# kuwt/edge_alignment

Hardware: NVIDIA B200
Metric: frame-pair alignments/sec at 640x480 (higher is better)
Workload: dtype f32+f64

## Files before the change

### edge_alignment_b200/csrc/ea_cabi.cu

```cuda
#include <cstdarg>
#include <cstdio>
#include <cstdlib>
#include <cmath>
#include <algorithm>
#include <cstring>
#include <mutex>
#include <vector>
#include <new>

#include "ea_internal.h"

thread_local std::string g_ea_err;
int ea_fail(int code, const char* fmt, ...) {
  char buf[512];
  va_list ap;
  va_start(ap, fmt);
  vsnprintf(buf, sizeof buf, fmt, ap);
  va_end(ap);
  g_ea_err = buf;
  return code;
}

int ea_ensure_tmp(ea_context* c, size_t bytes) {
  if (c->tmp_cap >= bytes) return EA_OK;
// ... 8 lines not shown
int ea_abi_version(void) { return EA_ABI_VERSION; }
const char* ea_last_error(void) { return g_ea_err.c_str(); }

int ea_create(int device, ea_context** out) {
  if (!out) return ea_fail(EA_ERR_INVALID_ARG, "ea_create: out is null");
  *out = nullptr;
  int n = 0;
  cudaError_t e = cudaGetDeviceCount(&n);
  if (e != cudaSuccess || n == 0)
    return ea_fail(EA_ERR_NO_DEVICE, "ea_create: no CUDA device (%s); this library has no CPU fallback", cudaGetErrorString(e));
  if (device < 0 || device >= n) return ea_fail(EA_ERR_INVALID_ARG, "ea_create: device %d out of range [0,%d)", device, n);
  CU(cudaSetDevice(device));
  cudaDeviceProp prop;
  CU(cudaGetDeviceProperties(&prop, device));
  if (prop.major < 10) return ea_fail(EA_ERR_NO_DEVICE, "ea_create: device %d is sm_%d%d; this build is sm_100a only", device, prop.major, prop.minor);
  ea_context* c = new (std::nothrow) ea_context();
  if (!c) return ea_fail(EA_ERR_INVALID_ARG, "out of host memory");
  struct Guard { ea_context* c; ~Guard() { if (c) ea_destroy(c); } } guard{c};
  c->device = device; c->sm_count = prop.multiProcessorCount; c->cc_major = prop.major; c->cc_minor = prop.minor;
  CU(cudaStreamCreateWithFlags(&c->stream, cudaStreamNonBlocking));
  c->own_stream = true;
  CU(cudaMalloc(&c->d_pose, 7 * sizeof(double)));
  CU(cudaMalloc(&c->d_failed, sizeof(int)));
  CU(cudaMalloc(&c->d_work, sizeof(int)));
  CU(cudaMalloc(&c->d_sums, size_t(1024) * EA_SUMS * sizeof(double)));
  {
    const char* h = getenv("EA_SOLVE_HELPERS");
    if (!(h && h[0] == '0')) {
      c->boards_bytes = ea_help_boards_bytes(c->sm_count);
      CU(cudaMalloc(&c->d_boards, c->boards_bytes));
    }
  }
  if (getenv("EA_SOLVE_DEBUG")) {
    CU(cudaMalloc(&c->d_debug, size_t(1024) * 6 * sizeof(unsigned long long)));
    CU(cudaMemset(c->d_debug, 0, size_t(1024) * 6 * sizeof(unsigned long long)));
  }
  guard.c = nullptr;
  *out = c;
  return EA_OK;
}
int ea_destroy(ea_context* c) {
  if (!c) return EA_OK;
  cudaSetDevice(c->device);
  cudaStreamSynchronize(c->stream);
  if (c->d_debug && c->debug_launches > 0) {
    const double n = double(c->debug_launches);
    fprintf(stderr, "[EA_SOLVE_DEBUG] %ld launches; per launch, mean over CTAs, kcycles of thread 0: eval %.1f  wait+totals %.1f  LM %.1f  wait2 %.1f  lifetime %.1f; evaluations %.1f\n",
            c->debug_launches, c->debug_sum[0] / n / 1e3, c->debug_sum[1] / n / 1e3, c->debug_sum[2] / n / 1e3, c->debug_sum[3] / n / 1e3, c->debug_sum[5] / n / 1e3, c->debug_sum[4] / n);
  }
  cudaFree(c->d_debug); cudaFree(c->d_boards); cudaFree(c->d_views);
  for (int k = 0; k < EA_PREP_MAX_PARTS; ++k) {
    if (c->prep_pipe.aux[k]) { cudaStreamSynchronize(c->prep_pipe.aux[k]); cudaStreamDestroy(c->prep_pipe.aux[k]); }
    if (c->prep_pipe.ev_front[k]) cudaEventDestroy(c->prep_pipe.ev_front[k]);
    if (c->prep_pipe.ev_dt[k]) cudaEventDestroy(c->prep_pipe.ev_dt[k]);
  }
  cudaFree(c->d_pose); cudaFree(c->d_failed); cudaFree(c->d_work); cudaFree(c->d_sums); cudaFree(c->d_idx); cudaFree(c->d_tmp);
  if (c->own_stream) cudaStreamDestroy(c->stream);
  delete c;
  return EA_OK;
}
int ea_sync(ea_context* c) {
  if (!c) return ea_fail(EA_ERR_INVALID_ARG, "null context");
  CU(cudaStreamSynchronize(c->stream));
  return EA_OK;
}
int ea_set_stream(ea_context* c, void* s) {
  if (!c) return ea_fail(EA_ERR_INVALID_ARG, "null context");
  if (c->own_stream) { cudaStreamSynchronize(c->stream); cudaStreamDestroy(c->stream); c->own_stream = false; }
  c->stream = static_cast<cudaStream_t>(s);
  return EA_OK;
}
int ea_device_info(ea_context* c, int* sm, int* maj, int* min_) {
  if (!c) return ea_fail(EA_ERR_INVALID_ARG, "null context");
  if (sm) *sm = c->sm_count;
  if (maj) *maj = c->cc_major;
  if (min_) *min_ = c->cc_minor;
  return EA_OK;
}
int ea_host_alloc(void** p, size_t bytes) {
  if (!p) return ea_fail(EA_ERR_INVALID_ARG, "null pointer");
  CU(cudaHostAlloc(p, bytes, cudaHostAllocDefault));
// ... 553 lines not shown
  if (e != cudaSuccess) return ea_fail(EA_ERR_CUDA, "gather probe: %s", cudaGetErrorString(e));
  CU(cudaEventElapsedTime(ms, ev.a, ev.b));
  std::vector<int32_t> slots(static_cast<size_t>(n));
  CU(cudaMemcpy(slots.data(), d_ref_slots, size_t(n) * sizeof(int32_t), cudaMemcpyDeviceToHost));
  std::vector<int> npts(size_t(ref->n_slots) * EA_MAX_LEVELS);
  CU(cudaMemcpy(npts.data(), ref->d_npts, npts.size() * sizeof(int), cudaMemcpyDeviceToHost));
  double total = 0.0;
  for (int i = 0; i < n; ++i) total += std::min(npts[size_t(slots[size_t(i)]) * EA_MAX_LEVELS + level], ref->lv[level].cap);
  *point_gathers = total * repeats;
  return EA_OK;
}

int ea_solve_batch_device_ordered(ea_context* c, int n, ea_frameset* ref, const int32_t* d_ref_slots, ea_frameset* now,
                                  const int32_t* d_now_slots, double* d_poses7, const int32_t* d_pose_index,
                                  const int32_t* d_order, const ea_solve_params* sp, ea_summary* d_summaries, bool tail_helpers) {
  if (!c || !d_ref_slots || !d_now_slots || !d_poses7) return ea_fail(EA_ERR_INVALID_ARG, "null argument");
  if (n <= 0) return EA_OK;
  EaSolveArgs A;
  int cluster = 0;
  int rc = fill_solve_args(c, ref, now, sp, A, &cluster);
  if (rc) return rc;
  CU(cudaSetDevice(c->device));
  A.ref_slots = d_ref_slots; A.now_slots = d_now_slots; A.pose_index = d_pose_index; A.poses = d_poses7;
  A.summaries = d_summaries; A.n_pairs = n; A.work_counter = c->d_work; A.order = d_order;
  EaProfileScope prof(c, 1);
  cudaError_t e;
  A.trace = c->d_trace; A.trace_count = c->d_trace_count; A.trace_cap = c->trace_cap;
  if (cluster == 0) cluster = auto_cluster(c, n, 0);
  A.debug = c->d_debug;
  A.boards = tail_helpers ? static_cast<EaHelpBoard*>(c->d_boards) : nullptr;
  e = ea_launch_solve_batch(A, cluster, c->sm_count, c->stream);
  if (c->d_debug && e == cudaSuccess) {
    const int grid = std::min(n, c->sm_count);
    std::vector<unsigned long long> h(size_t(grid) * 6);
    cudaStreamSynchronize(c->stream);
    cudaMemcpy(h.data(), c->d_debug, h.size() * sizeof(unsigned long long), cudaMemcpyDeviceToHost);
    for (int k = 0; k < 6; ++k) { double sum = 0; for (int b = 0; b < grid; ++b) sum += double(h[size_t(b) * 6 + k]); c->debug_sum[k] += sum / grid; }
    {
      std::vector<double> life(static_cast<size_t>(grid));
      double mean = 0.0;
      for (int b = 0; b < grid; ++b) { life[size_t(b)] = double(h[size_t(b) * 6 + 5]); mean += life[size_t(b)] / grid; }
      std::sort(life.begin(), life.end());
      if (c->debug_launches % 7 == 3)
        fprintf(stderr, "[EA_SOLVE_DEBUG] launch %ld: owner lifetimes (kcycles) mean %.0f  p50 %.0f  p75 %.0f  p90 %.0f  p97 %.0f  max %.0f\n", c->debug_launches,
                mean / 1e3, life[size_t(grid / 2)] / 1e3, life[size_t(grid * 3 / 4)] / 1e3, life[size_t(grid * 9 / 10)] / 1e3, life[size_t(grid * 97 / 100)] / 1e3, life[size_t(grid - 1)] / 1e3);
    }
    c->debug_launches++;
  }
  c->launches++;
  if (e != cudaSuccess) return ea_fail(EA_ERR_CUDA, "solve launch: %s", cudaGetErrorString(e));
  return EA_OK;
}
extern "C" {

int ea_solve_batch(ea_context* c, int n, ea_frameset* ref, const int32_t* ref_slots, ea_frameset* now, const int32_t* now_slots,
                   double* poses7, const ea_solve_params* sp, ea_summary* summaries) {
  if (!c || !ref_slots || !now_slots || !poses7) return ea_fail(EA_ERR_INVALID_ARG, "null argument");
  if (n <= 0) return EA_OK;
  int rc = check_pairable(ref, now);
  if (!rc) rc = check_slots(ref, std::min(n, ref->n_slots), ref_slots);
  if (rc) return rc;
  for (int i = 0; i < n; ++i) {
    if (ref_slots[i] < 0 || ref_slots[i] >= ref->n_slots || now_slots[i] < 0 || now_slots[i] >= now->n_slots)
      return ea_fail(EA_ERR_INVALID_ARG, "pair %d: slot out of range", i);
    double q2 = 0;
    for (int k = 0; k < 4; ++k) q2 += poses7[i * 7 + k] * poses7[i * 7 + k];
    if (!(q2 > 0.999999 && q2 < 1.000001)) return ea_fail(EA_ERR_INVALID_ARG, "pair %d: quaternion is not unit (|q|^2=%g)", i, q2);
  }
  CU(cudaSetDevice(c->device));
  const int L = ref->p.n_levels;
  const size_t bytes = size_t(n) * (2 * sizeof(int32_t) + 7 * sizeof(double)) + size_t(n) * L * sizeof(ea_summary) + 64;
  rc = ea_ensure_tmp(c, bytes);
  if (rc) return rc;
  char* base = (char*)c->d_tmp;
// ... 46 lines not shown
```

### edge_alignment_b200/csrc/ea_internal.h

```cpp
#pragma once
#include <cuda_runtime.h>

#include <string>
#include <vector>

#include "ea_device.cuh"

#include "ea_solve.cuh"

#define EA_TRACE_DOUBLES 6

struct EaSolveArgs {
  const EaLevelDesc* ref_desc;
  const EaLevelDesc* now_desc;
  const int32_t* ref_slots;
  const int32_t* now_slots;
  const int32_t* pose_index;
  const int32_t* order;
  double* poses;
  int* work_counter;
  struct EaHelpBoard* boards;
  unsigned long long* debug;
  ea_summary* summaries;
  double* trace;
  int* trace_count;
  int trace_cap;
  int n_pairs, n_levels, coarsest, finest;
  double inv_depth_scale;
  EaLevelGeom ref_geom[EA_MAX_LEVELS];
  EaLevelGeom now_geom[EA_MAX_LEVELS];
  int ref_cap[EA_MAX_LEVELS];
  ea_solve_params sp;
  EaEvalConsts loss;
};

cudaError_t ea_launch_solve_batch(const EaSolveArgs& A, int cluster_size, int sm_count, cudaStream_t stream);
size_t ea_help_boards_bytes(int sm_count);
cudaError_t ea_launch_gather_probe(const EaSolveArgs& A, int level, int slices, int repeats, float* d_sink, cudaStream_t stream);
int ea_probe_gather_device(ea_context* c, int n, ea_frameset* ref, const int32_t* d_ref_slots, ea_frameset* now, const int32_t* d_now_slots,
                           const double* d_poses7, int level, int repeats, float* ms, double* point_gathers);
cudaError_t ea_launch_eval_points(const EaLevelDesc& rd, const EaLevelDesc& nd, const EaLevelGeom& rg,
                                  const EaLevelGeom& ng, double inv_depth_scale, const ea_solve_params& sp,
                                  const double* d_pose7, int n_res, double* d_raw, double* d_res, double* d_jac,
// ... 36 lines not shown
  int zero_to_one;
  float depth_one;
  EaCannyCfg canny;
  EaScratch scratch;
};
#define EA_PREP_MAX_PARTS 4
struct EaPrepPipe {
  cudaStream_t aux[EA_PREP_MAX_PARTS] = {};
  cudaEvent_t ev_front[EA_PREP_MAX_PARTS] = {}, ev_dt[EA_PREP_MAX_PARTS] = {};
  bool ready = false;
};
cudaError_t ea_launch_preprocess(const EaPrepArgs& A, int sm_count, cudaStream_t stream, int* launches, const EaPrepPipe* pipe = nullptr);
__host__ __device__ inline float* ea_dt_origin(const EaPrepLevel& L, int slot) {
  return L.dt + size_t(slot) * L.dt_slot + size_t(EA_DT_PAD) * L.dt_pitch + EA_DT_PAD;
}
cudaError_t ea_launch_dt_normalized_copy(const float* origin, int pitch, const float2* affine, int w, int h, float* out, cudaStream_t stream);
cudaError_t ea_launch_dt_import(const float* src, float* origin, int w, int h, int pitch, cudaStream_t stream);
cudaError_t ea_launch_dt_fill_pad(const EaPrepLevel& L, const int32_t* d_slots, int n, cudaStream_t stream);
cudaError_t ea_launch_canny_level(const EaPrepArgs& A, int l, const uint8_t* bgr, const void* depth, size_t frame_stride_px,
                                  bool slot_indexed, const EaCannyCfg& cfg, const EaScratch& S, cudaStream_t stream, int* launches);
cudaError_t ea_launch_exact_edt_level(const EaPrepArgs& A, int l, const EaScratch& S, cudaStream_t stream, int* launches);
cudaError_t ea_launch_unpack_mask(const uint32_t* bits, int w, int h, int words, int median, uint8_t* out,
                                  cudaStream_t stream);

struct ea_context {
  int device = 0, sm_count = 0, cc_major = 0, cc_minor = 0;
  cudaStream_t stream = nullptr;
  bool own_stream = false;
  int64_t launches = 0;
  double* d_pose = nullptr;
  int* d_failed = nullptr;
  int* d_work = nullptr;
  void* d_boards = nullptr; size_t boards_bytes = 0;
  unsigned long long* d_debug = nullptr; double debug_sum[6] = {0, 0, 0, 0, 0, 0}; long debug_launches = 0;
  double* d_sums = nullptr;
  int32_t* d_idx = nullptr;
  size_t idx_cap = 0;
  void* d_tmp = nullptr;
  size_t tmp_cap = 0;
  void* d_views = nullptr; size_t views_cap = 0;
  EaPrepPipe prep_pipe;
  bool profile = false;
  double* d_trace = nullptr; int* d_trace_count = nullptr; int trace_cap = 0;
  std::vector<cudaEvent_t> ev[2];
};
struct EaProfileScope {
  ea_context* c; int kind; cudaStream_t s;
  EaProfileScope(ea_context* c_, int kind_, cudaStream_t s_ = nullptr) : c(c_), kind(kind_), s(s_ ? s_ : c_->stream) {
    if (c->profile) { cudaEvent_t e; cudaEventCreate(&e); cudaEventRecord(e, s); c->ev[kind].push_back(e); }
  }
  ~EaProfileScope() {
    if (c->profile) { cudaEvent_t e; cudaEventCreate(&e); cudaEventRecord(e, s); c->ev[kind].push_back(e); }
  }
};

struct ea_frameset {
  ea_context* ctx = nullptr;
  ea_frame_params p;
  int n_slots = 0;
  EaPrepLevel lv[EA_MAX_LEVELS];
  EaLevelGeom geom[EA_MAX_LEVELS];
  EaLevelDesc* d_desc = nullptr;
  std::vector<EaLevelDesc> h_desc;
  int* d_npts = nullptr;
  unsigned* d_minmax = nullptr;
  float2* d_affine = nullptr;
  int* d_overflow = nullptr;
// ... 45 lines not shown
```

### edge_alignment_b200/csrc/ea_solve.cu

```cuda
#include <cooperative_groups.h>

#include "ea_internal.h"
#include <cstdlib>

#include "ea_solve.cuh"

namespace cg = cooperative_groups;

#define EA_SOLVE_WARPS (EA_SOLVE_THREADS / 32)
#ifndef EA_SOLVE_MIN_CTAS
#define EA_SOLVE_MIN_CTAS 1
#endif
#define EA_CMD_EXIT 2

struct EaMsg {
  const void* pts;
  const float* dt;
  float2 affine;
  int n_res, level, pts_mode, cmd;
  int rev;
  int same;
  int nh, pad;
  EaPose P;
};
#define EA_MSG_FIXED_WORDS 5
static_assert(sizeof(EaMsg) % 8 == 0, "EaMsg is copied as 8-byte words");

#define EA_MAX_HELPERS (EA_MAX_CHUNKS - 1)
#define EA_BOARD_EXIT (~0ull)
#define EA_BOARD_SPIN_LIMIT (1ll << 22)
struct EaHelpBoard {
  unsigned long long word;
  int n_helpers;
  int busy;
  unsigned long long done[EA_MAX_HELPERS];
  double chunk[EA_MAX_CHUNKS][32];
  EaMsg msg;
};

struct alignas(2 * EA_STAGE_SLOT * 8) EaSolveSmem {
  uint2 stage[2][EA_STAGE_SLOT];
  EaSolveArgs args;
  EaMsg msg[2];
  double part[EA_MAX_CHUNKS][EA_SOLVE_WARPS][EA_NSUM];
  double cpart[EA_MAX_CHUNKS][EA_SOLVE_WARPS];
  double sums[EA_SUMS + 3];
  double cluster_sums[8][EA_SUMS + 3];
  EaLmState lm;
  int pair, level, truncated;
  unsigned long long help_epoch;
  int help_owner, help_index, help_fail;
  long long dbg[6], dbg_t, dbg_t0;
};

template <bool INL>
__device__ __forceinline__ void ea_boss_next_impl(const EaSolveArgs& A, EaSolveSmem& S, EaMsg& out, bool new_pair_needed) {
  for (;;) {
    if (new_pair_needed) {
      const int ticket = atomicAdd(A.work_counter, 1);
      if (ticket >= A.n_pairs) { out.cmd = EA_CMD_EXIT; S.pair = -1; return; }
      const int pair = A.order ? A.order[ticket] : ticket;
      S.pair = pair; S.level = A.coarsest;
      const int pi = A.pose_index ? A.pose_index[pair] : pair;
#pragma unroll 1
      for (int i = 0; i < 7; ++i) S.lm.x[i] = A.poses[size_t(pi) * 7 + i];
      new_pair_needed = false;
    }
    const int pair = S.pair, level = S.level;
    if (level < A.finest) {
      const int pi = A.pose_index ? A.pose_index[pair] : pair;
#pragma unroll 1
      for (int i = 0; i < 7; ++i) A.poses[size_t(pi) * 7 + i] = S.lm.x[i];
      new_pair_needed = true;
      continue;
    }
    const EaLevelDesc rd = A.ref_desc[size_t(A.ref_slots[pair]) * EA_MAX_LEVELS + level];
    const EaLevelDesc nd = A.now_desc[size_t(A.now_slots[pair]) * EA_MAX_LEVELS + level];
    const int n_pts = min(*rd.n_pts, A.ref_cap[level]);
    const int n_res = (n_pts + A.sp.point_stride - 1) / A.sp.point_stride;
    S.truncated = *rd.truncated;
    if (n_res == 0) {
      if (A.summaries) { ea_summary z = {}; z.termination = EA_TERM_SKIPPED_NO_POINTS; A.summaries[size_t(pair) * A.n_levels + level] = z; }
      S.level = level - 1;
      continue;
    }
    EaLmState& L = S.lm;
    L.phase = 0; L.iter = 0; L.accepted = 0; L.rejected = 0; L.invalid_run = 0; L.evals = 0; L.term = EA_TERM_NONE;
#pragma unroll 1
    for (int i = 0; i < 7; ++i) L.cand[i] = L.x[i];
    if (rd.pts_mode == EA_POINTS_XYZ) ea_pose_setup<true>(L.cand, A.ref_geom[level], A.now_geom[level], out.P);
    else ea_pose_setup<false>(L.cand, A.ref_geom[level], A.now_geom[level], out.P);
    out.pts = rd.pts; out.dt = nd.dt - ea_dt_origin_offset(nd.w); out.affine = *nd.dt_affine; out.n_res = n_res; out.level = level; out.pts_mode = rd.pts_mode; out.cmd = EA_CMD_EVAL; out.rev = 0; out.same = 0; out.nh = 0; out.pad = 0;
    return;
  }
}

__device__ __noinline__ void ea_boss_next(const EaSolveArgs& A, EaSolveSmem& S, EaMsg& out, bool new_pair_needed) { ea_boss_next_impl<false>(A, S, out, new_pair_needed); }

__device__ __forceinline__ void ea_boss_step_warp(const EaSolveArgs& A, EaSolveSmem& S, const EaMsg& cur, EaMsg& out, const int lane) {
  const int acc0 = S.lm.accepted, rej0 = S.lm.rejected;
#ifdef EA_LM_PROFILE
  const long long t_in = clock64();
#endif
  const int cmd = ea_lm_advance_warp(S.lm, S.sums, A.sp, lane);
#ifdef EA_LM_PROFILE
  __syncwarp();
  if (lane == 0) { S.lm.prof[6] += clock64() - t_in; S.lm.prof[7] += 1; }
  __syncwarp();
#endif
  if (A.trace && lane == 0) {
    const int k = (*A.trace_count)++;
    if (k < A.trace_cap) {
      double* r = A.trace + size_t(k) * EA_TRACE_DOUBLES;
      r[0] = cur.level; r[1] = S.lm.accepted + S.lm.rejected; r[2] = S.lm.cost; r[3] = S.sums[28]; r[4] = S.lm.radius;
      r[5] = S.lm.accepted > acc0 ? 1.0 : (S.lm.rejected > rej0 ? 0.0 : -1.0);
    }
  }
  if (cmd == EA_CMD_EVAL) {
    EaPose P;
    if (cur.pts_mode == EA_POINTS_XYZ) ea_pose_setup<true>(S.lm.cand, A.ref_geom[cur.level], A.now_geom[cur.level], P);
    else ea_pose_setup<false>(S.lm.cand, A.ref_geom[cur.level], A.now_geom[cur.level], P);
    if (lane < EA_MSG_FIXED_WORDS) reinterpret_cast<unsigned long long*>(&out)[lane] = reinterpret_cast<const unsigned long long*>(&cur)[lane];
    if (lane == 5) { out.rev = S.lm.evals & 1; out.same = 1; out.nh = 0; out.pad = 0; }
    if (lane == 0) out.P = P;
    __syncwarp();
    return;
  }
  if (lane == 0) {
    if (A.summaries) {
      const EaLmState& L = S.lm;
      ea_summary z;
      z.termination = L.term; z.iterations = L.iter; z.accepted = L.accepted; z.rejected = L.rejected;
      z.n_residuals = cur.n_res; z.evaluations = L.evals; z.initial_cost = L.initial_cost; z.final_cost = L.cost;
      z.truncated = S.truncated; z.reserved = 0;
      A.summaries[size_t(S.pair) * A.n_levels + cur.level] = z;
    }
    S.level = cur.level - 1;
    ea_boss_next(A, S, out, false);
  }
  __syncwarp();
}


__device__ __forceinline__ unsigned long long ea_ld_acquire(const unsigned long long* p) {
  unsigned long long v;
  asm volatile("ld.acquire.gpu.global.u64 %0, [%1];" : "=l"(v) : "l"(p) : "memory");
  return v;
}
__device__ __forceinline__ void ea_st_release(unsigned long long* p, unsigned long long v) {
  asm volatile("st.release.gpu.global.u64 [%0], %1;" ::"l"(p), "l"(v) : "memory");
}

template <int THREADS>
__device__ __forceinline__ void ea_eval_chunks(const EaSolveArgs& A, EaSolveSmem& S, const EaMsg& M, const EaPose& P, const int cb, const int ce,
                                               const int chunk, const bool pre_valid, const bool chain_next_eval) {
  const EaLevelGeom& ng = A.now_geom[M.level];
  const bool rev = EA_ALTERNATE_SWEEP && M.rev, nrev = EA_ALTERNATE_SWEEP ? !rev : rev;
  const int lo = cb * chunk, hi = min(ce * chunk, M.n_res);
  if (M.pts_mode == EA_POINTS_XYZ)
    ea_eval_slice<true, THREADS>(M.pts, M.dt, M.affine, ng, A.inv_depth_scale, A.loss, A.sp.point_stride, P, lo, hi, S.part[cb], S.cpart[cb], rev, nullptr, false, false, false,
                                 chunk / THREADS, THREADS / 32);
  else
    ea_eval_slice<false, THREADS>(M.pts, M.dt, M.affine, ng, A.inv_depth_scale, A.loss, A.sp.point_stride, P, lo, hi, S.part[cb], S.cpart[cb], rev, &S.stage[0][0], pre_valid, chain_next_eval, nrev,
                                  chunk / THREADS, THREADS / 32);
}

template <int THREADS, bool CLUSTER>
__global__ void __launch_bounds__(THREADS, EA_SOLVE_MIN_CTAS) ea_k_solve_batch(const __grid_constant__ EaSolveArgs A) {
  __shared__ EaSolveSmem S;
  cg::cluster_group cluster = cg::this_cluster();
  const unsigned crank = CLUSTER ? cluster.block_rank() : 0u;
  const unsigned csize = CLUSTER ? cluster.num_blocks() : 1u;
  const int tid = threadIdx.x, lane = tid & 31, warp = tid >> 5;
  const bool boss = (crank == 0 && tid == 0);
  const bool helpers_on = !CLUSTER && A.boards != nullptr;
  EaHelpBoard* const my_board = helpers_on ? A.boards + blockIdx.x : nullptr;
  auto sync_all = [&]() { if (CLUSTER) cluster.sync(); else __syncthreads(); };
  auto publish = [&](const EaMsg& m, unsigned slot) {
    for (unsigned r = 0; r < csize; ++r) {
      EaSolveSmem* Sr = CLUSTER ? cluster.map_shared_rank(&S, r) : &S;
      Sr->msg[slot] = m;
    }
  };
  unsigned g = 0;
  if (tid == 0) S.args = A;
  __syncthreads();
  if (boss) {
    EaMsg m;
    S.help_epoch = 0; S.help_fail = 0;
    ea_boss_next(S.args, S, m, true);
    if (helpers_on && m.cmd != EA_CMD_EXIT) { *reinterpret_cast<volatile int*>(&my_board->busy) = 1; __threadfence(); }
    publish(m, 0);
  }
  sync_all();
  const bool dbg_on = A.debug != nullptr && tid == 0;
  if (dbg_on) { for (int k = 0; k < 6; ++k) S.dbg[k] = 0; S.dbg_t0 = clock64(); S.dbg_t = S.dbg_t0; }
#ifdef EA_LM_PROFILE
  if (tid == 0) for (int k = 0; k < 8; ++k) S.lm.prof[k] = 0;
#endif
  auto lap = [&](int k) { if (dbg_on) { const long long t = clock64(); S.dbg[k] += t - S.dbg_t; S.dbg_t = t; } };
  for (;;) {
    const EaMsg& M = S.msg[g & 1];
    if (M.cmd == EA_CMD_EXIT) break;
    const EaPose P = M.P;
    int chunk = 0, K = 1, cb = 0;
    if (CLUSTER) {
      const int j0 = int((long long)M.n_res * crank / csize), j1 = int((long long)M.n_res * (crank + 1) / csize);
      const EaLevelGeom& ng = A.now_geom[M.level];
      const bool rev = EA_ALTERNATE_SWEEP && M.rev, nrev = EA_ALTERNATE_SWEEP ? !rev : rev;
      if (M.pts_mode == EA_POINTS_XYZ) ea_eval_slice<true, THREADS>(M.pts, M.dt, M.affine, ng, A.inv_depth_scale, A.loss, A.sp.point_stride, P, j0, j1, S.part[0], S.cpart[0], rev);
      else ea_eval_slice<false, THREADS>(M.pts, M.dt, M.affine, ng, A.inv_depth_scale, A.loss, A.sp.point_stride, P, j0, j1, S.part[0], S.cpart[0], rev, &S.stage[0][0], M.same != 0, true, nrev);
    } else {
      K = ea_chunking(M.n_res, THREADS, chunk);
      cb = (K * M.nh) / (M.nh + 1);
      ea_eval_chunks<THREADS>(A, S, M, P, cb, K, chunk, M.same != 0, true);
    }
    lap(0);
    __syncthreads();
    if (warp == 0) {
      if (CLUSTER) {
        const double tot = ea_cta_total<THREADS / 32>(S.part[0], S.cpart[0], lane);
        EaSolveSmem* S0 = cluster.map_shared_rank(&S, 0);
        if (lane < EA_SUMS) S0->cluster_sums[crank][lane] = tot;
      } else {
        double tot = 0.0;
        if (M.nh > 0) {
          int ok = 1;
          if (lane < M.nh) {
            long long spins = 0;
            while (ea_ld_acquire(&my_board->done[lane]) != S.help_epoch) {
              if (++spins > EA_BOARD_SPIN_LIMIT) { ok = 0; break; }
            }
          }
          ok = __all_sync(0xffffffffu, ok);
          __threadfence();
          if (!ok && lane == 0) S.help_fail = 1;
          for (int c = 0; c < cb; ++c) tot += __ldcg(&my_board->chunk[c][lane]);
        }
        {
          double ct[EA_MAX_CHUNKS];
#pragma unroll
          for (int c = 0; c < EA_MAX_CHUNKS; ++c) ct[c] = (c >= cb && c < K) ? ea_cta_total<THREADS / 32>(S.part[c], S.cpart[c], lane) : 0.0;
#pragma unroll
          for (int c = 0; c < EA_MAX_CHUNKS; ++c) if (c >= cb && c < K) tot += ct[c];
        }
        if (lane < EA_SUMS) S.sums[lane] = tot;
        if (lane == 27 && S.help_fail) S.sums[27] = 1.0;
        __syncwarp();
        lap(1);
        EaMsg& nm = S.msg[(g + 1) & 1];
        int reg = 0;
        if (helpers_on && lane == 31) reg = *reinterpret_cast<volatile int*>(&my_board->n_helpers);
        ea_boss_step_warp(S.args, S, M, nm, lane);
        reg = __shfl_sync(0xffffffffu, reg, 31);
        if (helpers_on) {
          int nh = 0;
          if (nm.cmd == EA_CMD_EVAL && reg > 0) {
            int ch2; const int K2 = ea_chunking(nm.n_res, THREADS, ch2);
            nh = min(min(reg, EA_MAX_HELPERS), K2 - 1);
          }
          if (lane == 0) { nm.nh = nh; if (nh != M.nh) nm.same = 0; }
          __syncwarp();
          if (nh > 0) {
            unsigned long long* dst = reinterpret_cast<unsigned long long*>(&my_board->msg);
            for (int i = lane; i < int(sizeof(EaMsg) / 8); i += 32) __stcg(dst + i, reinterpret_cast<const unsigned long long*>(&nm)[i]);
            __threadfence();
            __syncwarp();
            if (lane == 0) { S.help_epoch += 1; ea_st_release(&my_board->word, (S.help_epoch << 8) | (unsigned long long)nh); }
          }
          if (nm.cmd == EA_CMD_EXIT && lane == 0) {
            *reinterpret_cast<volatile int*>(&my_board->busy) = 0;
            __threadfence();
            ea_st_release(&my_board->word, EA_BOARD_EXIT);
          }
        }
        lap(2);
      }
    }
    if (CLUSTER) {
      cluster.sync();
      if (crank == 0 && warp == 0) {
        double s = 0.0;
        if (lane < EA_SUMS) for (unsigned r = 0; r < csize; ++r) s += S.cluster_sums[r][lane];
        if (lane < EA_SUMS) S.sums[lane] = s;
        __syncwarp();
        EaMsg& nm = S.msg[(g + 1) & 1];
        ea_boss_step_warp(S.args, S, M, nm, lane);
        for (unsigned r = 1; r < csize; ++r) {
          unsigned long long* dst = reinterpret_cast<unsigned long long*>(&cluster.map_shared_rank(&S, r)->msg[(g + 1) & 1]);
          for (int i = lane; i < int(sizeof(EaMsg) / 8); i += 32) dst[i] = reinterpret_cast<const unsigned long long*>(&nm)[i];
        }
      }
    }
    sync_all();
    lap(3);
    if (dbg_on) S.dbg[4] += 1;
    g += 1;
  }
#ifdef EA_LM_PROFILE
  if (dbg_on && blockIdx.x == 0 && S.dbg[4] > 0)
    printf("[EA_LM_PROFILE] CTA 0, %lld evaluations; cycles per evaluation: tests %lld, update %lld, build %lld, LDLT %lld, model %lld, plus+stores %lld | advance_warp mean %lld\n",
           S.dbg[4], S.lm.prof[0] / S.dbg[4], S.lm.prof[1] / S.dbg[4], S.lm.prof[2] / S.dbg[4], S.lm.prof[3] / S.dbg[4], S.lm.prof[4] / S.dbg[4], S.lm.prof[5] / S.dbg[4], S.lm.prof[6] / S.dbg[4]);
#endif
  if (dbg_on) {
    S.dbg[5] = clock64() - S.dbg_t0;
    for (int k = 0; k < 6; ++k) A.debug[size_t(blockIdx.x) * 6 + k] = (unsigned long long)S.dbg[k];
  }
  if (CLUSTER) { cluster.sync(); return; }
  if (!helpers_on) return;
  for (;;) {
    if (tid == 0) {
      int best = -1, best_n = EA_MAX_HELPERS, any_busy = 0;
      const int G = int(gridDim.x);
      for (int k = 1; k < G; ++k) {
        const int o = (int(blockIdx.x) + k) % G;
        if (!*reinterpret_cast<volatile int*>(&A.boards[o].busy)) continue;
        any_busy = 1;
        const int nreg = *reinterpret_cast<volatile int*>(&A.boards[o].n_helpers);
        if (nreg < best_n) { best_n = nreg; best = o; }
      }
      int idx = 0;
      if (best >= 0) {
        idx = atomicAdd(&A.boards[best].n_helpers, 1) + 1;
        if (idx > EA_MAX_HELPERS) { atomicSub(&A.boards[best].n_helpers, 1); best = -2; }
      }
      S.help_owner = best >= 0 ? best : (any_busy || best == -2 ? -2 : -1);
      S.help_index = idx;
    }
    __syncthreads();
    const int owner = S.help_owner, index = S.help_index;
    __syncthreads();
    if (owner == -1) break;
    if (owner == -2) { __nanosleep(2000); continue; }
    EaHelpBoard* const B = A.boards + owner;
    unsigned long long seen = 0;
    for (;;) {
      if (tid == 0) {
        unsigned long long w;
        long long spins = 0;
// ... 239 lines not shown
```

### edge_alignment_b200/csrc/ea_solve.cuh

```cuda
#pragma once
#include <cfloat>

#include "ea_device.cuh"

#ifndef EA_SOLVE_THREADS
#define EA_SOLVE_THREADS 512
#endif

#define EA_CMD_EVAL 0
#define EA_CMD_DONE 1


struct EaLmState {
  double x[7];
  double cand[7];
  double H[21], b[6];
  double scale[6], diag[6];
  double cost, initial_cost, radius, decrease_factor, model_cost_change;
  double dl_mu, dl_alpha, dl_step_norm, dl_grad[6], dl_gn[6];
  int phase, iter, accepted, rejected, invalid_run, reuse_diag, evals, term;
  int dl_reuse, pad;
#ifdef EA_LM_PROFILE
  long long prof[8];
#endif
};
#ifdef EA_LM_PROFILE
#define EA_LM_LAP(k) do { const long long t_ = clock64(); if (lane == 0) S.prof[k] += t_ - lm_t_; lm_t_ = t_; } while (0)
#else
#define EA_LM_LAP(k) do { } while (0)
#endif

__device__ inline void ea_quat_plus(const double* x, const double* d, double* out) {
  const double n2 = d[0] * d[0] + d[1] * d[1] + d[2] * d[2];
  if (n2 > 0.0) {
    double s, c;
    if (n2 < 0.01) {
      c = fma(n2, fma(n2, fma(n2, fma(n2, fma(n2, fma(n2, 1.0 / 479001600.0, -1.0 / 3628800.0), 1.0 / 40320.0), -1.0 / 720.0), 1.0 / 24.0), -0.5), 1.0);
      s = fma(n2, fma(n2, fma(n2, fma(n2, fma(n2, fma(n2, 1.0 / 6227020800.0, -1.0 / 39916800.0), 1.0 / 362880.0), -1.0 / 5040.0), 1.0 / 120.0), -1.0 / 6.0), 1.0);
    } else {
      const double n = sqrt(n2);
      s = sin(n) / n; c = cos(n);
    }
    const double q0 = c, q1 = s * d[0], q2 = s * d[1], q3 = s * d[2];
    out[0] = q0 * x[0] - q1 * x[1] - q2 * x[2] - q3 * x[3];
    out[1] = q0 * x[1] + q1 * x[0] + q2 * x[3] - q3 * x[2];
    out[2] = q0 * x[2] - q1 * x[3] + q2 * x[0] + q3 * x[1];
    out[3] = q0 * x[3] + q1 * x[2] - q2 * x[1] + q3 * x[0];
  } else {
    out[0] = x[0]; out[1] = x[1]; out[2] = x[2]; out[3] = x[3];
  }
}
__device__ inline void ea_pose_plus(const double* x, const double* d, double* out) {
  ea_quat_plus(x, d, out);
  out[4] = x[4] + d[3]; out[5] = x[5] + d[4]; out[6] = x[6] + d[5];
// ... 196 lines not shown
      if (sqrt(sn) <= sp.parameter_tolerance * (sqrt(xn) + sp.parameter_tolerance)) { S.term = EA_TERM_CONVERGENCE_PARAMETER; return EA_CMD_DONE; }
    }
    const double cost_change = S.cost - cand_cost;
    if (fabs(cost_change) <= sp.function_tolerance * S.cost) { S.term = EA_TERM_CONVERGENCE_FUNCTION; return EA_CMD_DONE; }
    const double rel = fail ? -DBL_MAX : cost_change / S.model_cost_change;
    if (rel > sp.min_relative_decrease) {
#pragma unroll
      for (int i = 0; i < 7; ++i) S.x[i] = S.cand[i];
#pragma unroll
      for (int k = 0; k < 21; ++k) S.H[k] = sums[k];
#pragma unroll
      for (int k = 0; k < 6; ++k) S.b[k] = sums[21 + k];
      S.cost = cand_cost;
      if (sp.trust_region_strategy == 0) {
        const double t = 2.0 * rel - 1.0;
        S.radius = fmin(sp.max_trust_region_radius, S.radius / fmax(1.0 / 3.0, 1.0 - t * t * t));
        S.decrease_factor = 2.0; S.reuse_diag = 0;
      } else {
        if (rel < 0.25) S.radius *= 0.5;
        if (rel > 0.75) S.radius = fmax(S.radius, 3.0 * S.dl_step_norm);
        S.dl_mu = fmax(1e-8, 2.0 * S.dl_mu / 10.0); S.dl_reuse = 0;
      }
      S.accepted++;
      if (ea_gradient_converged(S, sp.gradient_tolerance)) { S.term = EA_TERM_CONVERGENCE_GRADIENT; return EA_CMD_DONE; }
    } else {
      if (sp.trust_region_strategy == 0) { S.radius = S.radius / S.decrease_factor; S.decrease_factor *= 2.0; S.reuse_diag = 1; }
      else { S.radius *= 0.5; S.dl_reuse = 1; }
      S.rejected++;
    }
  }
  return ea_lm_propose(S, sp);
}

static __device__ __noinline__ int ea_lm_advance(EaLmState& S, const double* sums, const ea_solve_params& sp) { return ea_lm_advance_impl(S, sums, sp); }
static __device__ __noinline__ int ea_lm_propose_slow(EaLmState& S, const ea_solve_params& sp) { return ea_lm_propose(S, sp); }

__device__ __forceinline__ bool ea_ldlt_solve6_packed(double (&U)[21], const double (&bs)[6], double (&y)[6]) {
  double dinv[6];
  bool ok = true;
#pragma unroll
  for (int j = 0; j < 6; ++j) {
    double d = U[ea_tri(j, j)];
    double v[6];
#pragma unroll
    for (int k = 0; k < j; ++k) { v[k] = U[ea_tri(k, j)] * U[ea_tri(k, k)]; d = fma(-U[ea_tri(k, j)], v[k], d); }
    ok = ok && (d > 0.0) && isfinite(d);
    U[ea_tri(j, j)] = d;
    dinv[j] = 1.0 / d;
#pragma unroll
    for (int i = j + 1; i < 6; ++i) {
      double t = U[ea_tri(j, i)];
#pragma unroll
      for (int k = 0; k < j; ++k) t = fma(-U[ea_tri(k, i)], v[k], t);
      U[ea_tri(j, i)] = t * dinv[j];
    }
  }
#pragma unroll
  for (int i = 0; i < 6; ++i) {
    double t = bs[i];
#pragma unroll
    for (int k = 0; k < i; ++k) t = fma(-U[ea_tri(k, i)], y[k], t);
    y[i] = t;
  }
#pragma unroll
  for (int i = 0; i < 6; ++i) y[i] *= dinv[i];
#pragma unroll
  for (int i = 5; i >= 0; --i) {
    double t = y[i];
// ... 251 lines not shown
      *slot += double(ea_warp_transpose_reduce(A.acc, lane));
#pragma unroll
      for (int k = 0; k < EA_NSUM; ++k) A.acc[k] = 0.0f;
      if (it + 1 == it1 || (chunk_iters > 0 && ((it + 1) & (chunk_iters - 1)) == 0)) {
        const double c64 = ea_warp_sum(cost64);
        if (lane == 0) cpart[size_t(kc) * part_stride + warp] = c64;
        cost64 = 0.0;
      }
    }
  }
  if (it1 <= it0) { if (lane == 0) cpart[warp] = 0.0; }
  if (staged && prefetch_next) {
    const int rn = residual_of(next_reverse ? it_first_rev : 0, next_reverse);
    ea_cp_async_wait_all();
    if (rn >= j0 && rn < j1) ea_cp_async8(st0, pts8 + size_t(unsigned(rn)) * stride8);
    ea_cp_async_commit();
  }
}

#ifndef EA_MAX_CHUNKS
#define EA_MAX_CHUNKS 4
#endif
__device__ __forceinline__ int ea_chunking(const int n_res, const int threads, int& size) {
  const int unit = threads * EA_FLUSH_EVERY;
  const int nb = (n_res + unit - 1) / unit;
  int s = 0;
  while (((nb + (1 << s) - 1) >> s) > EA_MAX_CHUNKS) ++s;
  size = unit << s;
  return n_res > 0 ? (n_res + size - 1) / size : 1;
}

template <int WARPS>
__device__ __forceinline__ double ea_cta_total(const double (*part)[EA_NSUM], const double* cpart, int lane) {
  double s = 0.0;
  if (lane < 28) {
#pragma unroll
    for (int w2 = 0; w2 < WARPS; ++w2) s += part[w2][lane];
  } else if (lane == 28) {
#pragma unroll
    for (int w2 = 0; w2 < WARPS; ++w2) s += cpart[w2];
  }
  return s;
}
```

Before: 118,100.

## Warp-parallelize boss pair setup and cache per-level fields in shared memory

The boss work that picks the next pair and level now runs across a whole warp instead of thread 0. Lanes load the pose, precompute per-level descriptors into shared memory, and write poses back in parallel. The next-pair call moves out of the lane-0 branch, the cross-warp total reduction becomes branch-free, and finer-grained debug timers are added. The intent is to shorten the serial section between evaluations. In exchange, clock64 calls are added to the LM advance path, and these run on every call even when debugging is off.

Measured after the change: 118,500, median of 6. No clear change (+0.4%).

```diff
diff --git a/edge_alignment_b200/csrc/ea_cabi.cu b/edge_alignment_b200/csrc/ea_cabi.cu
--- a/edge_alignment_b200/csrc/ea_cabi.cu
+++ b/edge_alignment_b200/csrc/ea_cabi.cu
@@ -64,8 +64,8 @@
     }
   }
   if (getenv("EA_SOLVE_DEBUG")) {
-    CU(cudaMalloc(&c->d_debug, size_t(1024) * 6 * sizeof(unsigned long long)));
-    CU(cudaMemset(c->d_debug, 0, size_t(1024) * 6 * sizeof(unsigned long long)));
+    CU(cudaMalloc(&c->d_debug, size_t(1024) * EA_DBG_N * sizeof(unsigned long long)));
+    CU(cudaMemset(c->d_debug, 0, size_t(1024) * EA_DBG_N * sizeof(unsigned long long)));
   }
   guard.c = nullptr;
   *out = c;
@@ -77,8 +77,23 @@
   cudaStreamSynchronize(c->stream);
   if (c->d_debug && c->debug_launches > 0) {
     const double n = double(c->debug_launches);
-    fprintf(stderr, "[EA_SOLVE_DEBUG] %ld launches; per launch, mean over CTAs, kcycles of thread 0: eval %.1f  wait+totals %.1f  LM %.1f  wait2 %.1f  lifetime %.1f; evaluations %.1f\n",
-            c->debug_launches, c->debug_sum[0] / n / 1e3, c->debug_sum[1] / n / 1e3, c->debug_sum[2] / n / 1e3, c->debug_sum[3] / n / 1e3, c->debug_sum[5] / n / 1e3, c->debug_sum[4] / n);
+    const double* d = c->debug_sum;
+    const double ev = d[EA_DBG_EVALS] > 0 ? d[EA_DBG_EVALS] : 1.0;
+    fprintf(stderr, "[EA_SOLVE_DEBUG] %ld launches; per launch, mean over CTAs, kcycles of thread 0: eval %.1f  wait %.1f  totals %.1f  "
+            "LM %.1f (serial %.1f)  message %.1f  next %.1f  publication %.1f  wait2 %.1f  lifetime %.1f; evaluations %.1f\n",
+            c->debug_launches, d[EA_DBG_EVAL] / n / 1e3, d[EA_DBG_WAIT] / n / 1e3, d[EA_DBG_TOTALS] / n / 1e3, d[EA_DBG_LM] / n / 1e3,
+            d[EA_DBG_SERIAL] / n / 1e3, d[EA_DBG_MSG] / n / 1e3, d[EA_DBG_NEXT] / n / 1e3, d[EA_DBG_PUB] / n / 1e3, d[EA_DBG_WAIT2] / n / 1e3,
+            d[EA_DBG_LIFE] / n / 1e3, d[EA_DBG_EVALS] / n);
+    fprintf(stderr, "[EA_SOLVE_DEBUG] cycles per evaluation: eval %.0f  wait %.0f  totals %.0f  fast track %.0f  serial %.0f  message %.0f  "
+            "next %.0f  publication %.0f  wait2 %.0f  | serial section %.0f  lifetime %.0f\n",
+            d[EA_DBG_EVAL] / ev, d[EA_DBG_WAIT] / ev, d[EA_DBG_TOTALS] / ev, (d[EA_DBG_LM] - d[EA_DBG_SERIAL]) / ev, d[EA_DBG_SERIAL] / ev,
+            d[EA_DBG_MSG] / ev, d[EA_DBG_NEXT] / ev, d[EA_DBG_PUB] / ev, d[EA_DBG_WAIT2] / ev,
+            (d[EA_DBG_WAIT] + d[EA_DBG_TOTALS] + d[EA_DBG_LM] + d[EA_DBG_MSG] + d[EA_DBG_NEXT] + d[EA_DBG_PUB] + d[EA_DBG_WAIT2]) / ev, d[EA_DBG_LIFE] / ev);
+    fprintf(stderr, "[EA_SOLVE_DEBUG] calls per launch: serial state machine %.1f  message %.1f  next %.1f  publication %.1f; "
+            "cycles per call: serial %.0f  message %.0f  next %.0f  publication %.0f\n",
+            d[EA_DBG_SERIAL_N] / n, d[EA_DBG_MSG_N] / n, d[EA_DBG_NEXT_N] / n, d[EA_DBG_PUB_N] / n,
+            d[EA_DBG_SERIAL] / (d[EA_DBG_SERIAL_N] > 0 ? d[EA_DBG_SERIAL_N] : 1.0), d[EA_DBG_MSG] / (d[EA_DBG_MSG_N] > 0 ? d[EA_DBG_MSG_N] : 1.0),
+            d[EA_DBG_NEXT] / (d[EA_DBG_NEXT_N] > 0 ? d[EA_DBG_NEXT_N] : 1.0), d[EA_DBG_PUB] / (d[EA_DBG_PUB_N] > 0 ? d[EA_DBG_PUB_N] : 1.0));
   }
   cudaFree(c->d_debug); cudaFree(c->d_boards); cudaFree(c->d_views);
   for (int k = 0; k < EA_PREP_MAX_PARTS; ++k) {
@@ -698,14 +713,14 @@
   e = ea_launch_solve_batch(A, cluster, c->sm_count, c->stream);
   if (c->d_debug && e == cudaSuccess) {
     const int grid = std::min(n, c->sm_count);
-    std::vector<unsigned long long> h(size_t(grid) * 6);
+    std::vector<unsigned long long> h(size_t(grid) * EA_DBG_N);
     cudaStreamSynchronize(c->stream);
     cudaMemcpy(h.data(), c->d_debug, h.size() * sizeof(unsigned long long), cudaMemcpyDeviceToHost);
-    for (int k = 0; k < 6; ++k) { double sum = 0; for (int b = 0; b < grid; ++b) sum += double(h[size_t(b) * 6 + k]); c->debug_sum[k] += sum / grid; }
+    for (int k = 0; k < EA_DBG_N; ++k) { double sum = 0; for (int b = 0; b < grid; ++b) sum += double(h[size_t(b) * EA_DBG_N + k]); c->debug_sum[k] += sum / grid; }
     {
       std::vector<double> life(static_cast<size_t>(grid));
       double mean = 0.0;
-      for (int b = 0; b < grid; ++b) { life[size_t(b)] = double(h[size_t(b) * 6 + 5]); mean += life[size_t(b)] / grid; }
+      for (int b = 0; b < grid; ++b) { life[size_t(b)] = double(h[size_t(b) * EA_DBG_N + EA_DBG_LIFE]); mean += life[size_t(b)] / grid; }
       std::sort(life.begin(), life.end());
       if (c->debug_launches % 7 == 3)
         fprintf(stderr, "[EA_SOLVE_DEBUG] launch %ld: owner lifetimes (kcycles) mean %.0f  p50 %.0f  p75 %.0f  p90 %.0f  p97 %.0f  max %.0f\n", c->debug_launches,
diff --git a/edge_alignment_b200/csrc/ea_internal.h b/edge_alignment_b200/csrc/ea_internal.h
--- a/edge_alignment_b200/csrc/ea_internal.h
+++ b/edge_alignment_b200/csrc/ea_internal.h
@@ -9,6 +9,22 @@
 #include "ea_solve.cuh"
 
 #define EA_TRACE_DOUBLES 6
+
+enum {
+  EA_DBG_EVAL,
+  EA_DBG_WAIT,
+  EA_DBG_TOTALS,
+  EA_DBG_LM,
+  EA_DBG_SERIAL,
+  EA_DBG_MSG,
+  EA_DBG_NEXT,
+  EA_DBG_PUB,
+  EA_DBG_WAIT2,
+  EA_DBG_EVALS,
+  EA_DBG_SERIAL_N, EA_DBG_MSG_N, EA_DBG_NEXT_N, EA_DBG_PUB_N,
+  EA_DBG_LIFE,
+  EA_DBG_N
+};
 
 struct EaSolveArgs {
   const EaLevelDesc* ref_desc;
@@ -111,7 +127,7 @@
   int* d_failed = nullptr;
   int* d_work = nullptr;
   void* d_boards = nullptr; size_t boards_bytes = 0;
-  unsigned long long* d_debug = nullptr; double debug_sum[6] = {0, 0, 0, 0, 0, 0}; long debug_launches = 0;
+  unsigned long long* d_debug = nullptr; double debug_sum[EA_DBG_N] = {}; long debug_launches = 0;
   double* d_sums = nullptr;
   int32_t* d_idx = nullptr;
   size_t idx_cap = 0;
diff --git a/edge_alignment_b200/csrc/ea_solve.cu b/edge_alignment_b200/csrc/ea_solve.cu
--- a/edge_alignment_b200/csrc/ea_solve.cu
+++ b/edge_alignment_b200/csrc/ea_solve.cu
@@ -38,6 +38,13 @@
   EaMsg msg;
 };
 
+struct EaLevelFields {
+  const void* pts;
+  const float* dt;
+  float2 affine;
+  int n_res, pts_mode, truncated, pad;
+};
+
 struct alignas(2 * EA_STAGE_SLOT * 8) EaSolveSmem {
   uint2 stage[2][EA_STAGE_SLOT];
   EaSolveArgs args;
@@ -47,62 +54,85 @@
   double sums[EA_SUMS + 3];
   double cluster_sums[8][EA_SUMS + 3];
   EaLmState lm;
-  int pair, level, truncated;
+  int pair, level, truncated, pose_slot;
+  EaLevelFields lvl[EA_MAX_LEVELS];
   unsigned long long help_epoch;
   int help_owner, help_index, help_fail;
-  long long dbg[6], dbg_t, dbg_t0;
+  long long dbg[EA_DBG_N], dbg_t, dbg_t0;
 };
 
-template <bool INL>
-__device__ __forceinline__ void ea_boss_next_impl(const EaSolveArgs& A, EaSolveSmem& S, EaMsg& out, bool new_pair_needed) {
+__device__ __forceinline__ void ea_dbg_lap(EaSolveSmem& S, const bool on, const int k, const int kn = -1) {
+  if (on) { const long long t = clock64(); S.dbg[k] += t - S.dbg_t; S.dbg_t = t; if (kn >= 0) S.dbg[kn] += 1; }
+}
+
+__device__ __noinline__ void ea_boss_next(const EaSolveArgs& A, EaSolveSmem& S, EaMsg& out, bool new_pair_needed, const int lane) {
+  const unsigned full = 0xffffffffu;
   for (;;) {
     if (new_pair_needed) {
-      const int ticket = atomicAdd(A.work_counter, 1);
-      if (ticket >= A.n_pairs) { out.cmd = EA_CMD_EXIT; S.pair = -1; return; }
+      int ticket = 0;
+      if (lane == 0) ticket = atomicAdd(A.work_counter, 1);
+      ticket = __shfl_sync(full, ticket, 0);
+      if (ticket >= A.n_pairs) { if (lane == 0) { out.cmd = EA_CMD_EXIT; S.pair = -1; } __syncwarp(); return; }
       const int pair = A.order ? A.order[ticket] : ticket;
-      S.pair = pair; S.level = A.coarsest;
       const int pi = A.pose_index ? A.pose_index[pair] : pair;
-#pragma unroll 1
-      for (int i = 0; i < 7; ++i) S.lm.x[i] = A.poses[size_t(pi) * 7 + i];
+      const int rs = A.ref_slots[pair], ns = A.now_slots[pair];
+      double x = 0.0;
+      if (lane < 7) x = A.poses[size_t(pi) * 7 + lane];
+      const int l = lane - 8;
+      const bool mine = l >= 0 && l < EA_MAX_LEVELS && l >= A.finest && l <= A.coarsest;
+      EaLevelFields F = {};
+      if (mine) {
+        const EaLevelDesc rd = A.ref_desc[size_t(rs) * EA_MAX_LEVELS + l];
+        const EaLevelDesc nd = A.now_desc[size_t(ns) * EA_MAX_LEVELS + l];
+        const int n_pts = min(*rd.n_pts, A.ref_cap[l]);
+        F.pts = rd.pts; F.dt = nd.dt - ea_dt_origin_offset(nd.w); F.affine = *nd.dt_affine;
+        F.n_res = (n_pts + A.sp.point_stride - 1) / A.sp.point_stride; F.pts_mode = rd.pts_mode; F.truncated = *rd.truncated;
+      }
+      if (lane < 7) S.lm.x[lane] = x;
+      if (mine) S.lvl[l] = F;
+      if (lane == 0) { S.pair = pair; S.level = A.coarsest; S.pose_slot = pi; }
+      __syncwarp();
       new_pair_needed = false;
     }
     const int pair = S.pair, level = S.level;
     if (level < A.finest) {
-      const int pi = A.pose_index ? A.pose_index[pair] : pair;
-#pragma unroll 1
-      for (int i = 0; i < 7; ++i) A.poses[size_t(pi) * 7 + i] = S.lm.x[i];
+      if (lane < 7) A.poses[size_t(S.pose_slot) * 7 + lane] = S.lm.x[lane];
+      __syncwarp();
       new_pair_needed = true;
       continue;
     }
-    const EaLevelDesc rd = A.ref_desc[size_t(A.ref_slots[pair]) * EA_MAX_LEVELS + level];
-    const EaLevelDesc nd = A.now_desc[size_t(A.now_slots[pair]) * EA_MAX_LEVELS + level];
-    const int n_pts = min(*rd.n_pts, A.ref_cap[level]);
-    const int n_res = (n_pts + A.sp.point_stride - 1) / A.sp.point_stride;
-    S.truncated = *rd.truncated;
+    const EaLevelFields& F = S.lvl[level];
+    const int n_res = F.n_res;
     if (n_res == 0) {
-      if (A.summaries) { ea_summary z = {}; z.termination = EA_TERM_SKIPPED_NO_POINTS; A.summaries[size_t(pair) * A.n_levels + level] = z; }
-      S.level = level - 1;
+      if (lane == 0) {
+        if (A.summaries) { ea_summary z = {}; z.termination = EA_TERM_SKIPPED_NO_POINTS; A.summaries[size_t(pair) * A.n_levels + level] = z; }
+        S.level = level - 1;
+      }
+      __syncwarp();
       continue;
     }
     EaLmState& L = S.lm;
-    L.phase = 0; L.iter = 0; L.accepted = 0; L.rejected = 0; L.invalid_run = 0; L.evals = 0; L.term = EA_TERM_NONE;
-#pragma unroll 1
-    for (int i = 0; i < 7; ++i) L.cand[i] = L.x[i];
-    if (rd.pts_mode == EA_POINTS_XYZ) ea_pose_setup<true>(L.cand, A.ref_geom[level], A.now_geom[level], out.P);
-    else ea_pose_setup<false>(L.cand, A.ref_geom[level], A.now_geom[level], out.P);
-    out.pts = rd.pts; out.dt = nd.dt - ea_dt_origin_offset(nd.w); out.affine = *nd.dt_affine; out.n_res = n_res; out.level = level; out.pts_mode = rd.pts_mode; out.cmd = EA_CMD_EVAL; out.rev = 0; out.same = 0; out.nh = 0; out.pad = 0;
+    if (lane == 0) { L.phase = 0; L.iter = 0; L.accepted = 0; L.rejected = 0; L.invalid_run = 0; L.evals = 0; L.term = EA_TERM_NONE; S.truncated = F.truncated; }
+    if (lane < 7) L.cand[lane] = L.x[lane];
+    EaPose P;
+    if (F.pts_mode == EA_POINTS_XYZ) ea_pose_setup<true>(L.x, A.ref_geom[level], A.now_geom[level], P);
+    else ea_pose_setup<false>(L.x, A.ref_geom[level], A.now_geom[level], P);
+    if (lane == 0) {
+      out.P = P;
+      out.pts = F.pts; out.dt = F.dt; out.affine = F.affine; out.n_res = n_res; out.level = level; out.pts_mode = F.pts_mode; out.cmd = EA_CMD_EVAL; out.rev = 0; out.same = 0; out.nh = 0; out.pad = 0;
+    }
+    __syncwarp();
     return;
   }
 }
 
-__device__ __noinline__ void ea_boss_next(const EaSolveArgs& A, EaSolveSmem& S, EaMsg& out, bool new_pair_needed) { ea_boss_next_impl<false>(A, S, out, new_pair_needed); }
-
-__device__ __forceinline__ void ea_boss_step_warp(const EaSolveArgs& A, EaSolveSmem& S, const EaMsg& cur, EaMsg& out, const int lane) {
+__device__ __forceinline__ void ea_boss_step_warp(const EaSolveArgs& A, EaSolveSmem& S, const EaMsg& cur, EaMsg& out, const int lane, const bool dbg) {
   const int acc0 = S.lm.accepted, rej0 = S.lm.rejected;
 #ifdef EA_LM_PROFILE
   const long long t_in = clock64();
 #endif
   const int cmd = ea_lm_advance_warp(S.lm, S.sums, A.sp, lane);
+  ea_dbg_lap(S, A.debug != nullptr && lane == 0, EA_DBG_LM);
 #ifdef EA_LM_PROFILE
   __syncwarp();
   if (lane == 0) { S.lm.prof[6] += clock64() - t_in; S.lm.prof[7] += 1; }
@@ -124,6 +154,7 @@
     if (lane == 5) { out.rev = S.lm.evals & 1; out.same = 1; out.nh = 0; out.pad = 0; }
     if (lane == 0) out.P = P;
     __syncwarp();
+    ea_dbg_lap(S, A.debug != nullptr && lane == 0, EA_DBG_MSG, EA_DBG_MSG_N);
     return;
   }
   if (lane == 0) {
@@ -136,9 +167,10 @@
       A.summaries[size_t(S.pair) * A.n_levels + cur.level] = z;
     }
     S.level = cur.level - 1;
-    ea_boss_next(A, S, out, false);
   }
   __syncwarp();
+  ea_boss_next(A, S, out, false, lane);
+  ea_dbg_lap(S, A.debug != nullptr && lane == 0, EA_DBG_NEXT, EA_DBG_NEXT_N);
 }
 
 
@@ -172,33 +204,27 @@
   const unsigned crank = CLUSTER ? cluster.block_rank() : 0u;
   const unsigned csize = CLUSTER ? cluster.num_blocks() : 1u;
   const int tid = threadIdx.x, lane = tid & 31, warp = tid >> 5;
-  const bool boss = (crank == 0 && tid == 0);
   const bool helpers_on = !CLUSTER && A.boards != nullptr;
   EaHelpBoard* const my_board = helpers_on ? A.boards + blockIdx.x : nullptr;
   auto sync_all = [&]() { if (CLUSTER) cluster.sync(); else __syncthreads(); };
-  auto publish = [&](const EaMsg& m, unsigned slot) {
-    for (unsigned r = 0; r < csize; ++r) {
-      EaSolveSmem* Sr = CLUSTER ? cluster.map_shared_rank(&S, r) : &S;
-      Sr->msg[slot] = m;
-    }
-  };
   unsigned g = 0;
   if (tid == 0) S.args = A;
   __syncthreads();
-  if (boss) {
-    EaMsg m;
-    S.help_epoch = 0; S.help_fail = 0;
-    ea_boss_next(S.args, S, m, true);
-    if (helpers_on && m.cmd != EA_CMD_EXIT) { *reinterpret_cast<volatile int*>(&my_board->busy) = 1; __threadfence(); }
-    publish(m, 0);
+  if (crank == 0 && warp == 0) {
+    if (lane == 0) { S.help_epoch = 0; S.help_fail = 0; S.lm.serial_calls = 0; S.lm.serial_cycles = 0; }
+    ea_boss_next(S.args, S, S.msg[0], true, lane);
+    if (lane == 0) {
+      if (helpers_on && S.msg[0].cmd != EA_CMD_EXIT) { *reinterpret_cast<volatile int*>(&my_board->busy) = 1; __threadfence(); }
+      for (unsigned r = 1; r < csize; ++r) cluster.map_shared_rank(&S, r)->msg[0] = S.msg[0];
+    }
   }
   sync_all();
   const bool dbg_on = A.debug != nullptr && tid == 0;
-  if (dbg_on) { for (int k = 0; k < 6; ++k) S.dbg[k] = 0; S.dbg_t0 = clock64(); S.dbg_t = S.dbg_t0; }
+  if (dbg_on) { for (int k = 0; k < EA_DBG_N; ++k) S.dbg[k] = 0; S.dbg_t0 = clock64(); S.dbg_t = S.dbg_t0; }
 #ifdef EA_LM_PROFILE
   if (tid == 0) for (int k = 0; k < 8; ++k) S.lm.prof[k] = 0;
 #endif
-  auto lap = [&](int k) { if (dbg_on) { const long long t = clock64(); S.dbg[k] += t - S.dbg_t; S.dbg_t = t; } };
+  auto lap = [&](int k, int kn = -1) { ea_dbg_lap(S, dbg_on, k, kn); };
   for (;;) {
     const EaMsg& M = S.msg[g & 1];
     if (M.cmd == EA_CMD_EXIT) break;
@@ -215,13 +241,16 @@
       cb = (K * M.nh) / (M.nh + 1);
       ea_eval_chunks<THREADS>(A, S, M, P, cb, K, chunk, M.same != 0, true);
     }
-    lap(0);
+    lap(EA_DBG_EVAL);
     __syncthreads();
+    lap(EA_DBG_WAIT);
     if (warp == 0) {
       if (CLUSTER) {
         const double tot = ea_cta_total<THREADS / 32>(S.part[0], S.cpart[0], lane);
         EaSolveSmem* S0 = cluster.map_shared_rank(&S, 0);
         if (lane < EA_SUMS) S0->cluster_sums[crank][lane] = tot;
+        __syncwarp();
+        lap(EA_DBG_TOTALS);
       } else {
         double tot = 0.0;
         if (M.nh > 0) {
@@ -247,11 +276,11 @@
         if (lane < EA_SUMS) S.sums[lane] = tot;
         if (lane == 27 && S.help_fail) S.sums[27] = 1.0;
         __syncwarp();
-        lap(1);
+        lap(EA_DBG_TOTALS);
         EaMsg& nm = S.msg[(g + 1) & 1];
         int reg = 0;
         if (helpers_on && lane == 31) reg = *reinterpret_cast<volatile int*>(&my_board->n_helpers);
-        ea_boss_step_warp(S.args, S, M, nm, lane);
+        ea_boss_step_warp(S.args, S, M, nm, lane, dbg_on);
         reg = __shfl_sync(0xffffffffu, reg, 31);
         if (helpers_on) {
           int nh = 0;
@@ -274,7 +303,7 @@
             ea_st_release(&my_board->word, EA_BOARD_EXIT);
           }
         }
-        lap(2);
+        lap(EA_DBG_PUB, EA_DBG_PUB_N);
       }
     }
     if (CLUSTER) {
@@ -285,7 +314,7 @@
         if (lane < EA_SUMS) S.sums[lane] = s;
         __syncwarp();
         EaMsg& nm = S.msg[(g + 1) & 1];
-        ea_boss_step_warp(S.args, S, M, nm, lane);
+        ea_boss_step_warp(S.args, S, M, nm, lane, dbg_on);
         for (unsigned r = 1; r < csize; ++r) {
           unsigned long long* dst = reinterpret_cast<unsigned long long*>(&cluster.map_shared_rank(&S, r)->msg[(g + 1) & 1]);
           for (int i = lane; i < int(sizeof(EaMsg) / 8); i += 32) dst[i] = reinterpret_cast<const unsigned long long*>(&nm)[i];
@@ -293,18 +322,21 @@
       }
     }
     sync_all();
-    lap(3);
-    if (dbg_on) S.dbg[4] += 1;
+    lap(EA_DBG_WAIT2);
+    if (dbg_on) S.dbg[EA_DBG_EVALS] += 1;
     g += 1;
   }
 #ifdef EA_LM_PROFILE
-  if (dbg_on && blockIdx.x == 0 && S.dbg[4] > 0)
+  if (dbg_on && blockIdx.x == 0 && S.dbg[EA_DBG_EVALS] > 0) {
+    const long long ne = S.dbg[EA_DBG_EVALS];
     printf("[EA_LM_PROFILE] CTA 0, %lld evaluations; cycles per evaluation: tests %lld, update %lld, build %lld, LDLT %lld, model %lld, plus+stores %lld | advance_warp mean %lld\n",
-           S.dbg[4], S.lm.prof[0] / S.dbg[4], S.lm.prof[1] / S.dbg[4], S.lm.prof[2] / S.dbg[4], S.lm.prof[3] / S.dbg[4], S.lm.prof[4] / S.dbg[4], S.lm.prof[5] / S.dbg[4], S.lm.prof[6] / S.dbg[4]);
+           ne, S.lm.prof[0] / ne, S.lm.prof[1] / ne, S.lm.prof[2] / ne, S.lm.prof[3] / ne, S.lm.prof[4] / ne, S.lm.prof[5] / ne, S.lm.prof[6] / ne);
+  }
 #endif
   if (dbg_on) {
-    S.dbg[5] = clock64() - S.dbg_t0;
-    for (int k = 0; k < 6; ++k) A.debug[size_t(blockIdx.x) * 6 + k] = (unsigned long long)S.dbg[k];
+    S.dbg[EA_DBG_LIFE] = clock64() - S.dbg_t0;
+    S.dbg[EA_DBG_SERIAL] = S.lm.serial_cycles; S.dbg[EA_DBG_SERIAL_N] = S.lm.serial_calls;
+    for (int k = 0; k < EA_DBG_N; ++k) A.debug[size_t(blockIdx.x) * EA_DBG_N + k] = (unsigned long long)S.dbg[k];
   }
   if (CLUSTER) { cluster.sync(); return; }
   if (!helpers_on) return;
diff --git a/edge_alignment_b200/csrc/ea_solve.cuh b/edge_alignment_b200/csrc/ea_solve.cuh
--- a/edge_alignment_b200/csrc/ea_solve.cuh
+++ b/edge_alignment_b200/csrc/ea_solve.cuh
@@ -19,7 +19,9 @@
   double cost, initial_cost, radius, decrease_factor, model_cost_change;
   double dl_mu, dl_alpha, dl_step_norm, dl_grad[6], dl_gn[6];
   int phase, iter, accepted, rejected, invalid_run, reuse_diag, evals, term;
-  int dl_reuse, pad;
+  int dl_reuse;
+  int serial_calls;
+  long long serial_cycles;
 #ifdef EA_LM_PROFILE
   long long prof[8];
 #endif
@@ -282,8 +284,18 @@
   return ea_lm_propose(S, sp);
 }
 
-static __device__ __noinline__ int ea_lm_advance(EaLmState& S, const double* sums, const ea_solve_params& sp) { return ea_lm_advance_impl(S, sums, sp); }
-static __device__ __noinline__ int ea_lm_propose_slow(EaLmState& S, const ea_solve_params& sp) { return ea_lm_propose(S, sp); }
+static __device__ __noinline__ int ea_lm_advance(EaLmState& S, const double* sums, const ea_solve_params& sp) {
+  const long long t0 = clock64();
+  const int cmd = ea_lm_advance_impl(S, sums, sp);
+  S.serial_cycles += clock64() - t0; S.serial_calls++;
+  return cmd;
+}
+static __device__ __noinline__ int ea_lm_propose_slow(EaLmState& S, const ea_solve_params& sp) {
+  const long long t0 = clock64();
+  const int cmd = ea_lm_propose(S, sp);
+  S.serial_cycles += clock64() - t0; S.serial_calls++;
+  return cmd;
+}
 
 __device__ __forceinline__ bool ea_ldlt_solve6_packed(double (&U)[21], const double (&bs)[6], double (&y)[6]) {
   double dinv[6];
@@ -601,13 +613,11 @@
 
 template <int WARPS>
 __device__ __forceinline__ double ea_cta_total(const double (*part)[EA_NSUM], const double* cpart, int lane) {
+  const bool slot = lane < 28;
+  const double* src = slot ? &part[0][lane] : cpart;
+  const int stride = slot ? EA_NSUM : 1;
   double s = 0.0;
-  if (lane < 28) {
-#pragma unroll
-    for (int w2 = 0; w2 < WARPS; ++w2) s += part[w2][lane];
-  } else if (lane == 28) {
-#pragma unroll
-    for (int w2 = 0; w2 < WARPS; ++w2) s += cpart[w2];
-  }
-  return s;
-}
+#pragma unroll 4
+  for (int w2 = 0; w2 < WARPS; ++w2) s += src[w2 * stride];
+  return lane <= 28 ? s : 0.0;
+}
```
